# wvu-irl/flope

Hardware: AMD Instinct MI355X
Metric: poses_per_sec (higher is better)
Workload: dtype f16; 1 GPU; PoseResNet (ResNet-18 trunk + fp32 head) forward + special Procrustes + pose assembly, batch 256 x 224x224x3 16-bit NHWC crops resident in HBM per GPU (BASELINE configs[1]); one RCCL all-gather of the poses per run when N>1 (configs[3]); batch_per_gpu=256, global_batch=256, crop=224, parallelism=dp1, weights=synthetic_state_dict(seed 0), eval-mode BN folded

## Files before the change

flope_amd/csrc/conv_s1r.hip:

```cpp
#include "common.h"
#include "plan.h"
#include <type_traits>

namespace {

__device__ __forceinline__ void glds16(const char* gptr, unsigned lds_addr) {
  asm volatile("s_mov_b32 m0, %1\n\ts_nop 0\n\tglobal_load_lds_dwordx4 %0, off" ::"v"(gptr), "s"(lds_addr) : "memory");
}
#define GLDS16(gptr, lptr) glds16((gptr), (unsigned)__builtin_amdgcn_readfirstlane((int)(size_t)(__attribute__((address_space(3))) char*)(lptr)))

template <typename T, bool RES, bool FOLD>
__global__ __launch_bounds__(512, 1) void conv_s1r_kernel(const ConvP p, const u32x4* __restrict__ wpk) {
  static_assert(!(RES && FOLD), "the folded shortcut replaces the residual");
  typedef typename Elem<T>::frag frag;
  constexpr int NPT = 7, WO = 28;
  constexpr int PROW_B = 32 * 64;
  constexpr int IMG_B = 6 * PROW_B;
  constexpr int BUF_B = 4 * IMG_B;
  constexpr int SWAP_OFF = 2 * BUF_B;
  constexpr int NSTEP = 18;
  extern __shared__ __attribute__((aligned(16))) char smem[];

  const int tid = threadIdx.x, lane = tid & 63, wave = tid >> 6, g = lane >> 4, r16 = lane & 15;
  const int cg = wave & 3, kh = wave >> 2;
  const int G = gridDim.x, total = p.B * (p.Ho >> 2), rgs = p.Ho >> 2;

  int dso[4];
  {
    const int px = 16 * (wave & 1) + (lane >> 2);
#pragma unroll
    for (int k = 0; k < 4; ++k) dso[k] = min(px, WO + 1) * 256 + (wave >> 1) * 64 + (((lane & 3) ^ k) << 4);
  }
  const int wrow = p.Wip * 256;
  char* const dbase = smem + (wave >> 1) * IMG_B + (wave & 1) * 1024;
#define S1R_PIECE(src_, buf_, k_) GLDS16((src_) + (k_) * wrow + dso[(k_) & 3], dbase + (buf_) * BUF_B + (k_) * PROW_B)

  const int i8 = r16 < 4 ? r16 : (r16 < 12 ? r16 - 4 : r16 - 8);
  const int rr = i8 >> 1, cc = 2 * (i8 & 1) + ((r16 >= 4 && r16 < 12) ? 1 : 0);
  int rd[3];
#pragma unroll
  for (int dy = 0; dy < 3; ++dy) rd[dy] = kh * 2 * IMG_B + (rr + dy) * PROW_B + cc * 64 + ((g ^ ((rr + dy) & 3)) << 4);
  const int ooff = ((rr * p.Wop + cc) * p.Cout + 32 * cg + 8 * g) * 2;

#ifdef FLOPE_STAG_DBG
  const unsigned long long t_entry_ = __builtin_amdgcn_s_memtime(), rt_entry_ = __builtin_amdgcn_s_memrealtime();
#endif
  int tile = blockIdx.x;
  if (tile >= total) return;
  auto band = [&](int tl) -> const char* {
    tl = min(tl, total - 1);
    const int img = tl / rgs, rg = tl - img * rgs;
    return (const char*)p.in + ((size_t)img * p.Hip + 4 * rg) * p.Wip * 256;
  };
#pragma unroll
  for (int k = 0; k < 6; ++k) S1R_PIECE(band(tile), 0, k);

  const u32x4* const wl = wpk + (size_t)(cg * 2 + kh) * NSTEP * 2 * 64 + lane;
  frag wres[NSTEP][2];
  f32x4 b4[2];
#pragma unroll
  for (int s = 0; s < NSTEP; ++s)
#pragma unroll
    for (int ct = 0; ct < 2; ++ct) wres[s][ct] = __builtin_bit_cast(frag, wl[(s * 2 + ct) * 64]);
#pragma unroll
  for (int ct = 0; ct < 2; ++ct) b4[ct] = *(const f32x4*)(p.bias + 32 * cg + 8 * g + 4 * ct);
  frag wds[2];
  if constexpr (FOLD) {
#pragma unroll
    for (int ct = 0; ct < 2; ++ct) wds[ct] = __builtin_bit_cast(frag, ((const u32x4*)p.ds_w)[((cg * 2 + kh) * 2 + ct) * 64 + lane]);
#pragma unroll
    for (int ct = 0; ct < 2; ++ct) asm volatile("" : "+v"(wds[ct]));
  }
  const int xsoff = FOLD ? ((2 * rr + 1) * p.ds_Wip + 2 * cc + 1) * 128 + kh * 64 + g * 16 : 0;
#pragma unroll
  for (int s = 0; s < NSTEP; ++s)
#pragma unroll
    for (int ct = 0; ct < 2; ++ct) asm volatile("" : "+v"(wres[s][ct]));
#pragma unroll
  for (int ct = 0; ct < 2; ++ct) asm volatile("" : "+v"(b4[ct]));
  asm volatile("s_waitcnt vmcnt(0)" ::: "memory");
  __builtin_amdgcn_s_barrier();

#ifdef FLOPE_STAG_DBG
  const unsigned long long t_loop_ = __builtin_amdgcn_s_memtime();
#endif
  char* const swp = smem + SWAP_OFF + cg * (14 * 1024) + lane * 16;
  const f32x4 zero4 = {0.f, 0.f, 0.f, 0.f};
  int cur = 0;
  const char* nsrc = nullptr;
  const char* xsrc = nullptr;
  size_t opix = 0;

#ifdef FLOPE_STAG_DBG
  unsigned long long stp[12] = {0};
  int st_it = 0;
#define S1R_STAMP(i_) do { if ((p.dbg & 64) && st_it == 1) { __builtin_amdgcn_sched_barrier(0); stp[i_] = __builtin_amdgcn_s_memtime(); __builtin_amdgcn_sched_barrier(0); } } while (0)
#else
#define S1R_STAMP(i_) do {} while (0)
#endif
  auto sub = [&](auto kh_, auto p0_, auto np_) {
    constexpr int KH = decltype(kh_)::value, P0 = decltype(p0_)::value, NP = decltype(np_)::value;
    constexpr bool FIRST = P0 == 0;
    constexpr int NF = KH ? NP - 2 : 2, F0 = KH ? 2 : 0;
    constexpr int NS = NP - NF, S0 = KH ? 0 : 2;
    constexpr int WSLOT = (FIRST ? 0 : 8) + (KH ? (FIRST ? 4 : 2) : 0);
    constexpr int RSLOT = (FIRST ? 0 : 8) + (KH ? 0 : (FIRST ? 4 : 2));
    char* const obase = (char*)p.out + opix;
    const char* const rbase = RES ? (const char*)p.res + opix : nullptr;
    char* const xbuf = smem + cur * BUF_B + P0 * 256;
    const int nbuf = cur ^ 1;
    f32x4 acc[NP][2];
    frag xf[2][NP];
    frag xs[NP];
    S1R_STAMP(FIRST ? 0 : 5);
    auto xaddr = [&](int s) -> const char* {
      const int hc = s / 9, tap = s - 9 * hc, ky = tap / 3, kx = tap - 3 * ky;
      return xbuf + hc * IMG_B + rd[ky] + kx * 64;
    };
#pragma unroll
    for (int pt = 0; pt < NP; ++pt) xf[0][pt] = *(const frag*)(xaddr(0) + pt * 256);
    __builtin_amdgcn_sched_barrier(0);
#pragma unroll
    for (int s = 0; s < NSTEP; ++s) {
#pragma unroll
      for (int pt = 0; pt < NP; ++pt) {
#pragma unroll
        for (int ct = 0; ct < 2; ++ct)
          acc[pt][ct] = Elem<T>::mfma(wres[s][ct], xf[s & 1][pt], s == 0 ? (KH ? zero4 : b4[ct]) : acc[pt][ct]);
        if (s + 1 < NSTEP) xf[(s + 1) & 1][pt] = *(const frag*)(xaddr(s + 1) + pt * 256);
        if (FIRST && s < 3 && pt < 2) S1R_PIECE(nsrc, nbuf, 2 * s + pt);
        if (FOLD && s == 12) xs[pt] = *(const frag*)(xsrc + (P0 + pt) * 1024);
        __builtin_amdgcn_sched_group_barrier(0x008, 2, 0);
        if (s + 1 < NSTEP) __builtin_amdgcn_sched_group_barrier(0x100, 1, 0);
        if ((FIRST && s < 3 && pt < 2) || (FOLD && s == 12)) __builtin_amdgcn_sched_group_barrier(0x020, 1, 0);
      }
    }
    if constexpr (FOLD) {
#pragma unroll
      for (int pt = 0; pt < NP; ++pt)
#pragma unroll
        for (int ct = 0; ct < 2; ++ct) acc[pt][ct] = Elem<T>::mfma(wds[ct], xs[pt], acc[pt][ct]);
    }
    S1R_STAMP(FIRST ? 1 : 6);
#pragma unroll
    for (int i = 0; i < NS; ++i)
#pragma unroll
      for (int ct = 0; ct < 2; ++ct) *(f32x4*)(swp + ((WSLOT + i * 2 + ct) * 64) * 16) = acc[S0 + i][ct];
    u32x4 rq[NF];
    if constexpr (RES) {
#pragma unroll
      for (int i = 0; i < NF; ++i) rq[i] = *(const u32x4*)(rbase + (P0 + F0 + i) * 4 * p.Cout * 2);
    }
    __builtin_amdgcn_sched_barrier(0);
    if constexpr (!FIRST) { if constexpr (RES) asm volatile("s_waitcnt vmcnt(%0)" ::"n"(NF) : "memory"); else asm volatile("s_waitcnt vmcnt(0)" ::: "memory"); }
    asm volatile("s_waitcnt lgkmcnt(0)" ::: "memory");
    __builtin_amdgcn_sched_barrier(0);
    S1R_STAMP(FIRST ? 2 : 7);
#ifdef FLOPE_STAG_DBG
    if ((p.dbg & 64) && st_it == 1 && p.split_ws && lane == 0)
      ((unsigned long long*)p.split_ws)[8192 + (size_t)blockIdx.x * 16 + (FIRST ? 0 : 8) + wave] = __builtin_amdgcn_s_memtime();
#endif
    __builtin_amdgcn_s_barrier();
    __builtin_amdgcn_sched_barrier(0);
    asm volatile("" ::: "memory");
    S1R_STAMP(FIRST ? 3 : 8);
#pragma unroll
    for (int i = 0; i < NF; ++i) {
      u32x4 o;
#pragma unroll
      for (int ct = 0; ct < 2; ++ct) {
        const f32x4 pa = *(const f32x4*)(swp + ((RSLOT + i * 2 + ct) * 64) * 16);
        f32x4 v = KH ? pa + acc[F0 + i][ct] : acc[F0 + i][ct] + pa;
        if constexpr (RES) {
          v[0] += unpack_lo<T>(rq[i][2 * ct]); v[1] += unpack_hi<T>(rq[i][2 * ct]);
          v[2] += unpack_lo<T>(rq[i][2 * ct + 1]); v[3] += unpack_hi<T>(rq[i][2 * ct + 1]);
        }
        o[2 * ct] = pk_out16<T>(pack2<T>(v[0], v[1]), p.relu);
        o[2 * ct + 1] = pk_out16<T>(pack2<T>(v[2], v[3]), p.relu);
      }
      *(u32x4*)(obase + (P0 + F0 + i) * 4 * p.Cout * 2) = o;
    }
    __builtin_amdgcn_sched_barrier(0);
    S1R_STAMP(FIRST ? 4 : 9);
  };
  auto run = [&](auto kh_) {
    for (; tile < total; tile += G) {
      nsrc = band(tile + G);
      const int img = tile / rgs, rg = tile - img * rgs;
      if constexpr (FOLD) xsrc = (const char*)p.ds_in + ((size_t)img * p.ds_Hip + 8 * rg) * p.ds_Wip * 128 + xsoff;
      opix = (((size_t)img * p.Hop + 4 * rg + 1) * p.Wop + 1) * p.Cout * 2 + ooff;
      sub(kh_, std::integral_constant<int, 0>{}, std::integral_constant<int, 4>{});
      sub(kh_, std::integral_constant<int, 4>{}, std::integral_constant<int, 3>{});
#ifdef FLOPE_STAG_DBG
      if ((p.dbg & 64) && st_it == 1 && p.split_ws && tid == 0) {
        unsigned long long* d_ = (unsigned long long*)p.split_ws + (size_t)blockIdx.x * 16;
        for (int i = 0; i < 10; ++i) d_[i] = stp[i];
      }
      ++st_it;
#endif
      cur ^= 1;
    }
  };
  if (kh == 0) run(std::integral_constant<int, 0>{});
  else run(std::integral_constant<int, 1>{});
#ifdef FLOPE_STAG_DBG
  if ((p.dbg & 64) && p.split_ws && tid == 0) {
    unsigned long long* d_ = (unsigned long long*)p.split_ws + (size_t)blockIdx.x * 16;
    d_[10] = t_entry_; d_[11] = t_loop_; d_[12] = __builtin_amdgcn_s_memtime(); d_[13] = rt_entry_; d_[14] = __builtin_amdgcn_s_memrealtime();
  }
#endif
  asm volatile("s_waitcnt vmcnt(0)" ::: "memory");
#undef S1R_PIECE
#undef S1R_STAMP
}

}

extern "C" int flope_conv_s1r_ok(const ConvP* p) { return flope_plan::s1r_ok(flope_plan::dims_of(*p)); }

extern "C" int flope_conv_s1r_lds() { return (int)flope_plan::kS1rLds; }

extern "C" int flope_conv_s1r_init() {
  hipError_t e = hipSuccess;
#define A(T, R, F) if (e == hipSuccess) e = hipFuncSetAttribute((const void*)conv_s1r_kernel<T, R, F>, hipFuncAttributeMaxDynamicSharedMemorySize, flope_conv_s1r_lds());
  A(bf16_t, false, false) A(bf16_t, true, false) A(bf16_t, false, true) A(f16_t, false, false) A(f16_t, true, false) A(f16_t, false, true)
#undef A
  return (int)e;
}

extern "C" int flope_conv_s1r_launch(const ConvP* p, const void* w, int dtype, int grid, void* stream) {
  if (!flope_conv_s1r_ok(p) || !w) return (int)hipErrorInvalidValue;
  const int total = p->B * (p->Ho >> 2);
  if (grid > total) grid = total;
  if (grid < 1) return (int)hipErrorInvalidValue;
  const size_t lds = (size_t)flope_conv_s1r_lds();
  hipStream_t st = (hipStream_t)stream;
#define GO(T) do { if (p->ds_in) hipLaunchKernelGGL((conv_s1r_kernel<T, false, true>), dim3(grid), dim3(512), lds, st, *p, (const u32x4*)w);  \
                   else if (p->res) hipLaunchKernelGGL((conv_s1r_kernel<T, true, false>), dim3(grid), dim3(512), lds, st, *p, (const u32x4*)w);  \
                   else hipLaunchKernelGGL((conv_s1r_kernel<T, false, false>), dim3(grid), dim3(512), lds, st, *p, (const u32x4*)w); } while (0)
  if (dtype == 0) GO(bf16_t); else GO(f16_t);
#undef GO
  return (int)hipGetLastError();
}
```

flope_amd/csrc/engine.hip:

```cpp
#include "../../include/flope_amd.h"
#include "common.h"
#include "host_pack.h"
#include "plan.h"

#include <math.h>
#include <stdio.h>
#include <stdlib.h>
#include <string.h>

#include <map>
#include <string>
#include <vector>

extern "C" int flope_conv_mfma_init();
extern "C" int flope_conv_mfma_launch(const ConvP* p, int dtype, int cfg, int patch, int nbuf, size_t lds, void* stream);
extern "C" int flope_stem_init();
extern "C" int flope_stem_launch(const StemP* p, int dtype, size_t lds, void* stream);
extern "C" int flope_maxpool_launch(const PoolP* p, int dtype, void* stream);
extern "C" int flope_avgpool_launch(const void* in, float* out, int B, int h, int w, int C, int dtype, void* stream);
extern "C" int flope_fc1_launch(const float* feat, const float* W1, const float* W1p, const float* b1, float* hidden, int B, int K, int N, void* stream);
extern "C" int flope_fc2_procrustes_launch(const float* hidden, const float* W2, const float* b2, float* r9, float* R, int B, int K, const float* xyz, int nullify, float* Rt, void* stream);
extern "C" int flope_fc2_procrustes_k4_launch(const float* hidden, const float* W2, const float* b2, float* r9, float* R, int B, int K, const float* xyz, int nullify, float* Rt, void* stream);
extern "C" int flope_prep_input_launch(const void* x, int in_format, int B, int H, int W, void* out, int Hip, int Wip, int dtype, void* stream);
extern "C" int flope_read_stage_launch(const void* in, float* out, int B, int C, int h, int w, int dtype, void* stream);
extern "C" int flope_naive_conv_launch(const NaiveConvP* p, void* stream);
extern "C" int flope_conv_f32m_init();
extern "C" int flope_conv_f32m_launch(const F32mConvP* p, int mp, int stem, int grid, size_t lds, size_t ws_bytes, void* stream);
extern "C" int flope_conv_stag_init();
extern "C" int flope_conv_gstag_init();
extern "C" int flope_conv_w4_init();
extern "C" int flope_conv_r4_init();
extern "C" int flope_conv_r4_launch(const ConvP* p, int dtype, int grid_blocks, void* stream);
extern "C" int flope_conv_s1r_init();
extern "C" int flope_conv_s1r_launch(const ConvP* p, const void* w, int dtype, int grid, void* stream);
extern "C" int flope_conv_s2r_init();
extern "C" int flope_conv_s2r_launch(const ConvP* p, const void* w, int dtype, int grid, void* stream);
extern "C" int flope_conv_w4_launch(const ConvP* p, int dtype, int grid_blocks, int mt, void* stream);
extern "C" int flope_conv_gstag_launch(const ConvP* p, int dtype, void* stream);
extern "C" int flope_conv_stag_launch(const ConvP* p, int dtype, int grid_blocks, size_t lds, void* stream);
extern "C" int flope_conv_split_finalize_launch(const ConvP* p, int dtype, void* stream);
extern "C" int flope_stem_pool_init();
extern "C" int flope_stem_pool_r_blocks_per_cu();
#ifdef FLOPE_STAG_DBG
extern "C" void flope_stem_pool_set_dbg(void* ptr);
#endif
extern "C" int flope_stem_pool_launch(const void* x, int in_format, int B, int H, int W, int Hs, int Ws_, int Hq, int Wq,
                                      const void* w, const void* w2, int* queues, const float* bias, void* out, int dtype, int persist_blocks, void* stream);

using namespace flope_host;
using namespace flope_plan;

namespace {

thread_local std::string g_last_error;

constexpr double kBnEps = 1e-5;
constexpr size_t kDbgRegion = 1 << 20;
constexpr size_t kBufSlack = 1 << 20;

enum Image {
  kWPacked,
  kWStag,
  kWS2r,
  kWS1r,
  kWNaive,
  kWF32m,
  kBias,
  kWDsStag,
  kWDsS1r,
  kBiasFused,
  kImages
};

struct ConvDev {
  int in_buf = -1, out_buf = -1, res_buf = -1;
  int ip_in = -1, ip_out = -1, ip_res = -1;
  void* img[kImages] = {nullptr};
  Launch last;
};

struct Buf { void* ptr = nullptr; size_t bytes = 0; int C = 0, h = 0, w = 0; };

}

struct flope_engine {
  int device = 0, H = 0, W = 0, maxB = 0, dtype = 0, bod = 2048;
  int esz = 2;
  int num_cus = 256;
  PlanOptions opt;
  Plan plan;
  void* stem_in = nullptr; size_t stem_in_bytes = 0;
  int* stem_q = nullptr;
  void* stem_w = nullptr; void* stem_w2 = nullptr; float* stem_w_naive = nullptr; float* stem_w_f32m = nullptr; float* stem_bias = nullptr;
  std::vector<Buf> bufs;
  std::vector<ConvDev> convs;
  int stage_buf[10];
  int mid_buf[8];
  int ds_buf[3] = {-1, -1, -1}, ds_conv[3] = {-1, -1, -1};
  bool last_ds_folded[3] = {false, false, false};
  int final_buf = -1;
  int ip_final = -1;
  int stage_conv[10];
  int mid_conv[8];
  std::vector<int> ip_last_writer;
  bool ip_now = false;
  bool last_inplace = false;
  std::vector<int> last_ip_out, last_ip_writer;
  float *feat = nullptr, *hidden = nullptr, *W1 = nullptr, *W1p = nullptr, *b1 = nullptr, *W2 = nullptr, *b2 = nullptr;
  float* r9_scratch = nullptr;
  bool weights_loaded = false;
  float* split_ws = nullptr; size_t split_ws_bytes = 0;
  hipStream_t side[4] = {nullptr, nullptr, nullptr, nullptr};
  hipEvent_t ev_fork = nullptr, ev_join[4] = {nullptr, nullptr, nullptr, nullptr};
  std::vector<hipEvent_t> ev;
  int ev_n = 0;
  std::vector<int> ev_slice;
  int last_batch = 0;
// ... 434 lines not shown
  const bool fused = o.fuse_stem && dt != FLOPE_DT_F32;
  if (fused) {
    SMARK();
#ifdef FLOPE_STAG_DBG
    flope_stem_pool_set_dbg(((o.dbg & 64) && e->split_ws) ? (void*)(e->split_ws + (size_t)30 * (kDbgRegion / 4)) : nullptr);
#endif
    const bool stem_r = o.stem_r && e->stem_w2 && e->stem_q;
    K_TRY(e, "stem+maxpool", flope_stem_pool_launch(xs, in_format, batch, e->H, e->W, pl.Hs, pl.Ws, pl.Hq, pl.Wq, e->stem_w, stem_r ? e->stem_w2 : nullptr,
                                                   stem_r ? e->stem_q + 1024 * (x.slices > 1 ? x.slice : 0) : nullptr,
                                                   e->stem_bias, pool_out, dt,
                                                   stem_r ? flope_stem_pool_r_blocks_per_cu() * e->num_cus
                                                          : (o.stem_persist == 2 || (o.stem_persist == 1 && pl.Hq * pl.Wq <= 64 * 64)) ? 2 * e->num_cus : 0,
                                                   stream));
  } else {
    SMARK();
    K_TRY(e, "prep_input", flope_prep_input_launch(xs, in_format, batch, e->H, e->W, stem_in, pl.sHip, pl.sWip, dt, stream));
    if (dt == FLOPE_DT_F32 && o.f32mfma) {
      const Launch L = f32m_stem_launch(pl, x);
      F32mConvP p; memset(&p, 0, sizeof(p));
      p.in = (const float*)stem_in; p.out = (float*)stem_out; p.w = e->stem_w_f32m; p.bias = e->stem_bias;
      p.B = batch; p.Hip = pl.sHip; p.Wip = pl.sWip; p.Cin_stored = 4; p.Cin = 3; p.Ho = pl.Hs; p.Wo = pl.Ws;
      p.Hop = pl.Hs + 2; p.Wop = pl.Ws + 2; p.Cout = 64; p.KH = 7; p.KW = 7; p.stride = 2; p.in_off = 0; p.relu = 1;
      p.M = batch * pl.Hs * pl.Ws; p.nsteps = kF32mStemSteps;
      fastdiv_magic((unsigned)(pl.Hs * pl.Ws), &p.mg_hw, &p.sh_hw);
      fastdiv_magic((unsigned)pl.Ws, &p.mg_w, &p.sh_w);
      SMARK();
      K_TRY(e, "stem (fp32 MFMA)", flope_conv_f32m_launch(&p, L.mt, 1, L.grid, L.lds_bytes, 0, stream));
    } else if (dt == FLOPE_DT_F32) {
      NaiveConvP p; memset(&p, 0, sizeof(p));
      p.in = (const float*)stem_in; p.out = (float*)stem_out; p.w = e->stem_w_naive; p.bias = e->stem_bias;
      p.B = batch; p.Hip = pl.sHip; p.Wip = pl.sWip; p.Cin_stored = 4; p.Cin = 3; p.Ho = pl.Hs; p.Wo = pl.Ws;
      p.Hop = pl.Hs + 2; p.Wop = pl.Ws + 2; p.Cout = 64; p.KH = 7; p.KW = 7; p.stride = 2; p.in_off = 0; p.relu = 1;
      SMARK();
      K_TRY(e, "stem (fp32)", flope_naive_conv_launch(&p, stream));
    } else {
      StemP p; memset(&p, 0, sizeof(p));
      p.in = stem_in; p.out = stem_out; p.w = e->stem_w; p.bias = e->stem_bias;
      p.B = batch; p.Hip = pl.sHip; p.Wip = pl.sWip; p.Ho = pl.Hs; p.Wo = pl.Ws;
      p.tiles_per_image = pl.stem_tiles; p.patch_rows_max = pl.stem_rows;
      SMARK();
      K_TRY(e, "stem", flope_stem_launch(&p, dt, pl.stem_lds, stream));
    }
    PoolP pp; pp.in = stem_out; pp.out = pool_out; pp.B = batch; pp.Hip = pl.Hs + 2; pp.Wip = pl.Ws + 2; pp.C = 64; pp.Ho = pl.Hq; pp.Wo = pl.Wq;
    SMARK();
    K_TRY(e, "maxpool", flope_maxpool_launch(&pp, dt, stream));
  }
  for (size_t i = 0; i < e->convs.size(); ++i) {
    ConvDev& c = e->convs[i];
    const ConvShape& s = pl.shape[i];
    const Launch L = decide(o, pl, (int)i, x);
    if (x.slice == x.slices - 1) c.last = L;
    ConvP p, pf;
    if (L.family != kFolded && L.family != kNaive && L.family != kF32m) conv_params(e, (int)i, L, start, batch, &p, &pf);
    if (L.family != kFolded) SMARK();
    switch (L.family) {
      case kFolded: break;
      case kNaive: {
        NaiveConvP q; memset(&q, 0, sizeof(q));
        q.in = (const float*)buf_at(e, in_of(e, c), start); q.out = (float*)buf_at(e, out_of(e, c), start);
        q.res = res_of(e, c) >= 0 ? (const float*)buf_at(e, res_of(e, c), start) : nullptr;
        q.w = (const float*)c.img[kWNaive]; q.bias = (const float*)c.img[kBias];
        q.B = batch; q.Hip = s.hin + 2; q.Wip = s.win + 2; q.Cin_stored = s.cin; q.Cin = s.cin; q.Ho = s.hout; q.Wo = s.wout;
        q.Hop = s.hout + 2; q.Wop = s.wout + 2; q.Cout = s.cout; q.KH = s.k; q.KW = s.k; q.stride = s.stride;
        q.in_off = s.k == 3 ? 0 : 1; q.relu = s.relu;
        K_TRY(e, conv_name(s).c_str(), flope_naive_conv_launch(&q, stream));
        break;
      }
      case kF32m: {
        F32mConvP q; memset(&q, 0, sizeof(q));
        q.in = (const float*)buf_at(e, in_of(e, c), start); q.out = (float*)buf_at(e, out_of(e, c), start);
        q.res = res_of(e, c) >= 0 ? (const float*)buf_at(e, res_of(e, c), start) : nullptr;
        q.w = (const float*)c.img[kWF32m]; q.bias = (const float*)c.img[kBias];
        q.B = batch; q.Hip = s.hin + 2; q.Wip = s.win + 2; q.Cin_stored = s.cin; q.Cin = s.cin; q.Ho = s.hout; q.Wo = s.wout;
        q.Hop = s.hout + 2; q.Wop = s.wout + 2; q.Cout = s.cout; q.KH = s.k; q.KW = s.k; q.stride = s.stride;
        q.in_off = s.k == 3 ? 0 : 1; q.relu = s.relu;
        q.M = batch * s.hout * s.wout; q.csteps = s.cin / 16; q.nsteps = f32m_steps(s.cin, s.k);
        fastdiv_magic((unsigned)(s.hout * s.wout), &q.mg_hw, &q.sh_hw);
        fastdiv_magic((unsigned)s.wout, &q.mg_w, &q.sh_w);
        if (L.ksplit > 1) { q.ksplit = L.ksplit; q.split_ws = e->split_ws; }
        K_TRY(e, conv_name(s).c_str(), flope_conv_f32m_launch(&q, L.mt, 0, L.grid, L.lds_bytes, e->split_ws_bytes, stream));
        break;
      }
      case kGstag: K_TRY(e, conv_name(s).c_str(), flope_conv_gstag_launch(&p, dt, stream)); break;
      case kS1r: K_TRY(e, conv_name(s).c_str(), flope_conv_s1r_launch(&p, c.img[kWS1r], dt, L.grid, stream)); break;
      case kR4: K_TRY(e, conv_name(s).c_str(), flope_conv_r4_launch(&p, dt, L.grid, stream)); break;
      case kW4: K_TRY(e, conv_name(s).c_str(), flope_conv_w4_launch(&p, dt, L.grid, L.mt, stream)); break;
      case kStagFlat: case kStag512x64: case kStagBands:
        K_TRY(e, conv_name(s).c_str(), flope_conv_stag_launch(&p, dt, L.grid, L.lds_bytes, stream));
        if (L.ksplit > 1) K_TRY(e, conv_name(s).c_str(), flope_conv_split_finalize_launch(&pf, dt, stream));
        break;
      case kS2r: K_TRY(e, conv_name(s).c_str(), flope_conv_s2r_launch(&p, c.img[kWS2r], dt, L.grid, stream)); break;
      case kMfma: K_TRY(e, conv_name(s).c_str(), flope_conv_mfma_launch(&p, dt, L.cfg, L.patch, L.nbuf, L.lds_bytes, stream)); break;
    }
  }
  const int final_buf = e->ip_now ? e->ip_final : e->final_buf;
  const Buf& bl = e->bufs[final_buf];
  SMARK();
  K_TRY(e, "avgpool", flope_avgpool_launch(buf_at(e, final_buf, start), feat, batch, bl.h, bl.w, 512, dt, stream));
  SMARK();
  K_TRY(e, "fc1", flope_fc1_launch(feat, e->W1, o.fc1_packed ? e->W1p : nullptr, e->b1, hidden, batch, 512, e->bod, stream));
  if (head) {
    SMARK();
    float* r9 = (r9_dev ? r9_dev : e->r9_scratch) + (size_t)start * 9;
    float* Rp = R_dev ? R_dev + (size_t)start * 9 : nullptr;
    const float* xyzp = po.xyz ? po.xyz + (size_t)start * 3 : nullptr;
    float* Rtp = po.Rt ? po.Rt + (size_t)start * 16 : nullptr;
    int k4 = 0;
    if (o.fc2_k4) {
      k4 = flope_fc2_procrustes_k4_launch(hidden, e->W2, e->b2, r9, Rp, batch, e->bod, xyzp, po.nullify, Rtp, stream);
      if (k4 < 0) return fail(e, FLOPE_EHIP, "fc_rot+procrustes: launch failed");
    }
    if (!k4) K_TRY(e, "fc_rot+procrustes", flope_fc2_procrustes_launch(hidden, e->W2, e->b2, r9, Rp, batch, e->bod, xyzp, po.nullify, Rtp, stream));
  }
  SMARK();
#undef SMARK
  return FLOPE_OK;
}

static int run_trunk(flope_engine* e, const void* x_dev, int in_format, int batch, void* stream, bool head = false,
                     float* r9_dev = nullptr, float* R_dev = nullptr, const PoseOut& po = PoseOut()) {
  if (!e->weights_loaded) return fail(e, FLOPE_ESTATE, "forward before flope_load_weights");
  if (!x_dev) return fail(e, FLOPE_EINVAL, "forward: x_dev is NULL");
  if (batch < 1 || batch > e->maxB) return fail(e, FLOPE_EINVAL, "forward: batch must be within 1..max_batch");
  if (in_format < 0 || in_format > 3) return fail(e, FLOPE_EINVAL, "forward: unknown input format");
  HIP_TRY(e, hipSetDevice(e->device));
  e->ev_n = 0;
  e->last_fused = e->opt.fuse_stem && e->dtype != FLOPE_DT_F32;
  e->last_batch = batch;
  for (int i = 0; i < 3; ++i) e->last_ds_folded[i] = e->ds_conv[i] >= 0 && e->plan.conv[e->ds_conv[i]].folded;
  e->ip_now = e->last_inplace = e->opt.inplace != 0;
  if (e->ip_now) {
    e->last_ip_out.resize(e->convs.size());
    for (size_t i = 0; i < e->convs.size(); ++i) e->last_ip_out[i] = e->convs[i].ip_out;
    e->last_ip_writer = e->ip_last_writer;
  }
  const Slices sl = slices(e->opt, batch, e->opt.profile);
  const int ns = sl.n;
  if (ns == 1) return run_slice(e, x_dev, in_format, 0, slice_ctx(sl, 0, batch, e->num_cus), stream, true, head, r9_dev, R_dev, po);
  hipStream_t user = (hipStream_t)stream;
  if (e->opt.profile == 2) MARK(e, user, 0);
  HIP_TRY(e, hipEventRecord(e->ev_fork, user));
  const int first_side = e->opt.inline0 ? 1 : 0;
  const bool marks = e->opt.profile == 2;
  int rc_all = FLOPE_OK, forked = first_side;
  for (int s = first_side; s < ns && rc_all == FLOPE_OK; ++s) {
    if (hipStreamWaitEvent(e->side[s], e->ev_fork, 0) != hipSuccess) { rc_all = fail(e, FLOPE_EHIP, "hipStreamWaitEvent(fork) failed"); break; }

    forked = s + 1;
    if (e->opt.lag && !e->opt.inline0 && s == ns - 1 && batch >= 192) {
      hipLaunchKernelGGL(lag_kernel, dim3(1), dim3(64), 0, e->side[s], e->opt.lag);
      if (hipGetLastError() != hipSuccess) { rc_all = fail(e, FLOPE_EHIP, "lag kernel launch failed"); break; }
    }
    rc_all = run_slice(e, x_dev, in_format, sl.start[s], slice_ctx(sl, s, batch, e->num_cus), e->side[s], marks, head, r9_dev, R_dev, po);
  }
  if (e->opt.inline0 && rc_all == FLOPE_OK)
    rc_all = run_slice(e, x_dev, in_format, sl.start[0], slice_ctx(sl, 0, batch, e->num_cus), user, marks, head, r9_dev, R_dev, po);
  const std::string first_err = rc_all != FLOPE_OK ? e->err : std::string();
  for (int s = first_side; s < forked; ++s) {
    if (hipEventRecord(e->ev_join[s], e->side[s]) != hipSuccess || hipStreamWaitEvent(user, e->ev_join[s], 0) != hipSuccess) {
      hipStreamSynchronize(e->side[s]);
      if (rc_all == FLOPE_OK) rc_all = fail(e, FLOPE_EHIP, "joining the batch-slice streams failed");
    }
  }
  if (rc_all != FLOPE_OK) {
    if (!first_err.empty()) { e->err = first_err; g_last_error = first_err; }
    e->last_batch = 0;
  }
// ... 120 lines not shown
```

flope_amd/csrc/plan.h:

```cpp
#pragma once

#include "../../include/flope_amd.h"
#include "w4_sched.h"

#include <limits.h>
#include <stdio.h>
#include <string.h>

#include <algorithm>
#include <string>
#include <vector>

namespace flope_plan {

constexpr size_t kLdsTwoBlocks = 80 * 1024;
constexpr size_t kLdsMax = 160 * 1024;
constexpr size_t kGstagLds = 3 * 32768 + 3 * 16384;
constexpr size_t kR4Lds = (size_t)2 * 5 * 8192 + 18 * 4096 + 4 * 2048;
constexpr size_t kS1rLds = 2 * 4 * 6 * 32 * 64 + 4 * 14 * 1024;
constexpr size_t kS2rLds = 2 * 18 * 32 * 128;
constexpr size_t kF32mLds = kLdsTwoBlocks + 4096;

struct PlanOptions {
  int patch = 1;
  int bm256 = 1;
  int persist = 0;
  int rows_grid = 0;
  int split = 0;
  int fc1_packed = 1;
  int w4mtlo = 0;
  int lag = 20;
  int w4mt = 0;
  int fc2_k4 = 1;
  int ksplit = 1;
  int stem_r = 1;
  int stem_persist = 1;
  int rowseg = 1;
  int skew = 1;
  int r4 = 1;
  int s1r = 1;
  int s2r_grid = 0;
  int s2r = 1;
  int w4 = 1;
  int w4cw = 4;
  int w4cwf = 0;
  int prio = 0;
  int reslds = 1;
  int gstag = 1;
  int dsfuse = 1;
  int stag = 3;
  int streams = 2;
  int fuse_stem = 1;
  int ldspad = 0;
  int dbg = 0;
  int nbuf = 2;
  int f32mfma = 0;
  int f32m_ksplit = 0;
  int inline0 = 1;
  int inplace = 0;
  int profile = 0;
};

enum OptionKind { kBool, kClamp, kMask, kInOrZero, kZeroOrClamp, kNbuf };
struct OptionDef { const char* name; int PlanOptions::*member; OptionKind kind; int lo, hi; bool replans; };

inline const std::vector<OptionDef>& option_table() {
  typedef PlanOptions O;
  static const std::vector<OptionDef> t = {
      {"patch", &O::patch, kBool, 0, 1, true},
      {"bm256", &O::bm256, kBool, 0, 1, true},
      {"persist", &O::persist, kBool, 0, 1, false},
      {"rows_grid", &O::rows_grid, kClamp, -1, INT_MAX, false},
      {"split", &O::split, kClamp, 0, INT_MAX, false},
      {"fc1_packed", &O::fc1_packed, kBool, 0, 1, false},
      {"w4mtlo", &O::w4mtlo, kZeroOrClamp, 5, 8, false},
      {"lag", &O::lag, kClamp, 0, 500, false},
      {"w4mt", &O::w4mt, kInOrZero, 5, 8, false},
      {"fc2_k4", &O::fc2_k4, kBool, 0, 1, false},
      {"ksplit", &O::ksplit, kClamp, 0, 2, false},
      {"stem_r", &O::stem_r, kBool, 0, 1, false},
      {"stem_persist", &O::stem_persist, kClamp, 0, 2, false},
      {"rowseg", &O::rowseg, kBool, 0, 1, true},
      {"skew", &O::skew, kBool, 0, 1, true},
      {"r4", &O::r4, kBool, 0, 1, false},
      {"s1r", &O::s1r, kBool, 0, 1, false},
      {"s2r_grid", &O::s2r_grid, kClamp, INT_MIN, INT_MAX, false},
      {"s2r", &O::s2r, kBool, 0, 1, false},
      {"w4", &O::w4, kBool, 0, 1, false},
      {"w4cw", &O::w4cw, kClamp, 0, 64, false},
      {"w4cwf", &O::w4cwf, kMask, 0, 3, false},
      {"prio", &O::prio, kClamp, 0, 2, false},
      {"reslds", &O::reslds, kBool, 0, 1, false},
      {"gstag", &O::gstag, kClamp, 0, 2, true},
      {"dsfuse", &O::dsfuse, kBool, 0, 1, true},
      {"stag", &O::stag, kClamp, 0, 3, true},
      {"streams", &O::streams, kClamp, 1, 4, false},
      {"fuse_stem", &O::fuse_stem, kBool, 0, 1, false},
      {"ldspad", &O::ldspad, kClamp, INT_MIN, INT_MAX, false},
      {"dbg", &O::dbg, kClamp, INT_MIN, INT_MAX, false},
      {"nbuf", &O::nbuf, kNbuf, 2, 3, true},
      {"profile", &O::profile, kClamp, 0, 2, false},
      {"f32mfma", &O::f32mfma, kBool, 0, 1, false},
      {"f32m_ksplit", &O::f32m_ksplit, kClamp, 0, 32, false},
      {"inline0", &O::inline0, kBool, 0, 1, false},
      {"inplace", &O::inplace, kBool, 0, 1, false},
  };
  return t;
}

inline const OptionDef* find_option(const char* name) {
  for (const OptionDef& d : option_table())
    if (std::string(d.name) == name) return &d;
  return nullptr;
}

inline int set_option(PlanOptions& o, const char* name, int value, bool* replan) {
  const OptionDef* d = find_option(name);
  if (replan) *replan = d && d->replans;
  if (!d) return FLOPE_EINVAL;
  const int prev = o.*(d->member);
  const int clamped = value < d->lo ? d->lo : (value > d->hi ? d->hi : value);
  int v = clamped;
  switch (d->kind) {
    case kBool: v = value != 0; break;
    case kClamp: break;
    case kMask: v = value & d->hi; break;
    case kInOrZero: v = clamped == value ? value : 0; break;
    case kZeroOrClamp: v = value <= 0 ? 0 : clamped; break;
    case kNbuf: v = value == 2 ? 2 : 3; break;
  }
  o.*(d->member) = v;
  return prev;
}

enum ConvRole { kConv1, kShortcut, kConv2 };
struct ConvShape {
  int li = 0, bi = 0, role = kConv1;
  int cin = 0, cout = 0, k = 0, stride = 1;
  int hin = 0, win = 0, hout = 0, wout = 0;
  int res = 0;
  int relu = 0;
};

inline std::string conv_name(const ConvShape& s, bool bn = false) {
  const std::string p = "base.layer" + std::to_string(s.li) + "." + std::to_string(s.bi);
  if (s.role == kShortcut) return p + (bn ? ".downsample.1" : ".downsample.0");
  return p + (bn ? ".bn" : ".conv") + (s.role == kConv1 ? "1" : "2");
}

inline bool has_stag_image(const ConvShape& s) { return s.k == 3 && s.cin % 64 == 0; }
inline bool has_s1r_image(const ConvShape& s) { return s.k == 3 && s.stride == 1 && s.cin == 128 && s.cout == 128; }
inline bool has_s2r_image(const ConvShape& s) { return s.k == 3 && s.stride == 2 && s.cin == 64 && s.cout == 128; }
inline bool has_ds_s1r_image(const ConvShape& s) { return s.k == 1 && s.stride == 2 && s.cin == 64 && s.cout == 128; }
inline bool has_ds_stag_image(const ConvShape& s) { return s.k == 1 && s.cout >= 128 && s.cin % 64 == 0; }

inline int out_dim(int n, int k, int s, int p) { return (n + 2 * p - k) / s + 1; }

struct ConvDims {
  int stride, ntaps, Cin, Cout, Ho, Wo, Hip, Wip, ksplit;
  bool res, ds, ds_w;
  int ds_Cin, ds_Hip, ds_Wip;
};
template <typename P>
inline ConvDims dims_of(const P& p) {
  return {p.stride, p.ntaps, p.Cin, p.Cout, p.Ho, p.Wo, p.Hip, p.Wip, p.ksplit, p.res != nullptr, p.ds_in != nullptr, p.ds_w != nullptr,
          p.ds_Cin, p.ds_Hip, p.ds_Wip};
}
inline bool r4_ok(const ConvDims& p) {
  return p.stride == 1 && p.ntaps == 9 && p.Cin == 64 && p.Cout == 64 && p.Wo == 56 && p.Ho % 8 == 0 &&
         10 * (p.Wip + 2) * 4 <= 5 * 512 && p.ksplit <= 1 && !p.ds;
}
inline bool s1r_ok(const ConvDims& p) {
  if (p.ds && !(p.ds_Cin == 64 && p.ds_Hip == 2 * p.Ho + 2 && p.ds_Wip == 2 * p.Wo + 2 && p.ds_w && !p.res)) return false;
  return p.stride == 1 && p.ntaps == 9 && p.Cin == 128 && p.Cout == 128 && p.Wo == 28 && (p.Ho & 3) == 0 &&
         p.ksplit <= 1 && p.Wip == p.Wo + 2 && p.Hip == p.Ho + 2;
}
inline bool s2r_ok(const ConvDims& p) {
  return p.stride == 2 && p.ntaps == 9 && p.Cin == 64 && p.Cout == 128 && p.Wo == 28 && (p.Ho & 3) == 0 && !p.res && !p.ds &&
         p.ksplit <= 1 && p.Wip == 2 * p.Wo + 2 && p.Hip == 2 * p.Ho + 2;
}
inline size_t w4_lds(int pt, int mt, int dsf, int pers) {
  if (pt < 4 || pt > 6 || mt < 5 || mt > 8 || (mt < 7 && pt != 4) || (pers && (mt != 7 || pt > 5))) return 0;
  return w4_lds_bytes(pt, dsf && pers);
}

struct ConvPlan {
  int cfg = 0, patch = 0, nbuf = 2, per_image = 0, tiles_per_image = 0, ntiles = 0, rows_max = 0;
  size_t lds = 0;
// ... 482 lines not shown
```

Measured before the change: 275,900 poses/s.

## Peel first tile in s1r conv to stream weights and move prefetch to kh=1 waves

Adds a YW template mode to the stride-1 resident conv kernel and makes mode 2 the default. In that mode the first tile is peeled so only the first few weight steps are loaded before the loop, and the rest (plus the fused downsample weights) stream in during the first tile's MFMA steps. This is meant to hide the cold-start weight-load latency. The next band's prefetch is also moved out of the interleaved MFMA loop into one 12-piece burst issued by the kh=1 waves, which drops the vmcnt wait for kh=0 waves. The cost is more template variants, a more complex schedule, and possible register-pressure or ordering hazards in the peeled path.

After: 278,900 poses/s (median of 6 runs). 1.01x the previous value.

```diff
diff --git a/flope_amd/csrc/conv_s1r.hip b/flope_amd/csrc/conv_s1r.hip
--- a/flope_amd/csrc/conv_s1r.hip
+++ b/flope_amd/csrc/conv_s1r.hip
@@ -9,7 +9,7 @@
 }
 #define GLDS16(gptr, lptr) glds16((gptr), (unsigned)__builtin_amdgcn_readfirstlane((int)(size_t)(__attribute__((address_space(3))) char*)(lptr)))
 
-template <typename T, bool RES, bool FOLD>
+template <typename T, bool RES, bool FOLD, int YW>
 __global__ __launch_bounds__(512, 1) void conv_s1r_kernel(const ConvP p, const u32x4* __restrict__ wpk) {
   static_assert(!(RES && FOLD), "the folded shortcut replaces the residual");
   typedef typename Elem<T>::frag frag;
@@ -19,6 +19,8 @@
   constexpr int BUF_B = 4 * IMG_B;
   constexpr int SWAP_OFF = 2 * BUF_B;
   constexpr int NSTEP = 18;
+  constexpr bool PEEL = YW == 2;
+  constexpr int WD = 4;
   extern __shared__ __attribute__((aligned(16))) char smem[];
 
   const int tid = threadIdx.x, lane = tid & 63, wave = tid >> 6, g = lane >> 4, r16 = lane & 15;
@@ -34,6 +36,10 @@
   const int wrow = p.Wip * 256;
   char* const dbase = smem + (wave >> 1) * IMG_B + (wave & 1) * 1024;
 #define S1R_PIECE(src_, buf_, k_) GLDS16((src_) + (k_) * wrow + dso[(k_) & 3], dbase + (buf_) * BUF_B + (k_) * PROW_B)
+  const int ypx0 = (lane >> 2) * 256 + (wave & 3) * 64, ypx1 = min(16 + (lane >> 2), WO + 1) * 256 + (wave & 3) * 64, ysl = (lane & 3) << 4;
+  char* const ybase = smem + (wave & 3) * IMG_B;
+#define S1R_YPIECE(src_, buf_, q_) GLDS16((src_) + ((q_) >> 1) * wrow + (((q_) & 1) ? ypx1 : ypx0) + (ysl ^ ((((q_) >> 1) & 3) << 4)), \
+                                          ybase + (buf_) * BUF_B + ((q_) >> 1) * PROW_B + ((q_) & 1) * 1024)
 
   const int i8 = r16 < 4 ? r16 : (r16 < 12 ? r16 - 4 : r16 - 8);
   const int rr = i8 >> 1, cc = 2 * (i8 & 1) + ((r16 >= 4 && r16 < 12) ? 1 : 0);
@@ -54,31 +60,46 @@
   };
 #pragma unroll
   for (int k = 0; k < 6; ++k) S1R_PIECE(band(tile), 0, k);
+  if constexpr (PEEL) asm volatile("s_waitcnt vmcnt(0)" ::: "memory");
 
   const u32x4* const wl = wpk + (size_t)(cg * 2 + kh) * NSTEP * 2 * 64 + lane;
   frag wres[NSTEP][2];
   f32x4 b4[2];
-#pragma unroll
-  for (int s = 0; s < NSTEP; ++s)
+  if constexpr (PEEL) {
+#pragma unroll
+    for (int ct = 0; ct < 2; ++ct) b4[ct] = *(const f32x4*)(p.bias + 32 * cg + 8 * g + 4 * ct);
+  }
+#pragma unroll
+  for (int s = 0; s < (PEEL ? WD : NSTEP); ++s)
 #pragma unroll
     for (int ct = 0; ct < 2; ++ct) wres[s][ct] = __builtin_bit_cast(frag, wl[(s * 2 + ct) * 64]);
-#pragma unroll
-  for (int ct = 0; ct < 2; ++ct) b4[ct] = *(const f32x4*)(p.bias + 32 * cg + 8 * g + 4 * ct);
+  if constexpr (!PEEL) {
+#pragma unroll
+    for (int ct = 0; ct < 2; ++ct) b4[ct] = *(const f32x4*)(p.bias + 32 * cg + 8 * g + 4 * ct);
+  }
   frag wds[2];
-  if constexpr (FOLD) {
-#pragma unroll
-    for (int ct = 0; ct < 2; ++ct) wds[ct] = __builtin_bit_cast(frag, ((const u32x4*)p.ds_w)[((cg * 2 + kh) * 2 + ct) * 64 + lane]);
+  const u32x4* const wdl = FOLD ? (const u32x4*)p.ds_w + (size_t)(cg * 2 + kh) * 2 * 64 + lane : nullptr;
+  if constexpr (FOLD && !PEEL) {
+#pragma unroll
+    for (int ct = 0; ct < 2; ++ct) wds[ct] = __builtin_bit_cast(frag, wdl[ct * 64]);
 #pragma unroll
     for (int ct = 0; ct < 2; ++ct) asm volatile("" : "+v"(wds[ct]));
   }
   const int xsoff = FOLD ? ((2 * rr + 1) * p.ds_Wip + 2 * cc + 1) * 128 + kh * 64 + g * 16 : 0;
-#pragma unroll
-  for (int s = 0; s < NSTEP; ++s)
-#pragma unroll
-    for (int ct = 0; ct < 2; ++ct) asm volatile("" : "+v"(wres[s][ct]));
-#pragma unroll
-  for (int ct = 0; ct < 2; ++ct) asm volatile("" : "+v"(b4[ct]));
-  asm volatile("s_waitcnt vmcnt(0)" ::: "memory");
+  auto settle = [&]() {
+    if constexpr (FOLD && PEEL) {
+#pragma unroll
+      for (int ct = 0; ct < 2; ++ct) asm volatile("" : "+v"(wds[ct]));
+    }
+#pragma unroll
+    for (int s = 0; s < NSTEP; ++s)
+#pragma unroll
+      for (int ct = 0; ct < 2; ++ct) asm volatile("" : "+v"(wres[s][ct]));
+#pragma unroll
+    for (int ct = 0; ct < 2; ++ct) asm volatile("" : "+v"(b4[ct]));
+  };
+  if constexpr (!PEEL) { settle(); asm volatile("s_waitcnt vmcnt(0)" ::: "memory"); }
+  __builtin_amdgcn_sched_barrier(0);
   __builtin_amdgcn_s_barrier();
 
 #ifdef FLOPE_STAG_DBG
@@ -98,9 +119,11 @@
 #else
 #define S1R_STAMP(i_) do {} while (0)
 #endif
-  auto sub = [&](auto kh_, auto p0_, auto np_) {
+  auto sub = [&](auto kh_, auto p0_, auto np_, auto peeled_) {
     constexpr int KH = decltype(kh_)::value, P0 = decltype(p0_)::value, NP = decltype(np_)::value;
     constexpr bool FIRST = P0 == 0;
+    constexpr bool YHEAD = decltype(peeled_)::value ? !FIRST : FIRST;
+    constexpr bool WLOAD = decltype(peeled_)::value && FIRST;
     constexpr int NF = KH ? NP - 2 : 2, F0 = KH ? 2 : 0;
     constexpr int NS = NP - NF, S0 = KH ? 0 : 2;
     constexpr int WSLOT = (FIRST ? 0 : 8) + (KH ? (FIRST ? 4 : 2) : 0);
@@ -119,6 +142,10 @@
     };
 #pragma unroll
     for (int pt = 0; pt < NP; ++pt) xf[0][pt] = *(const frag*)(xaddr(0) + pt * 256);
+    if constexpr (YW >= 1 && KH == 1 && YHEAD) {
+#pragma unroll
+      for (int q = 0; q < 12; ++q) S1R_YPIECE(nsrc, nbuf, q);
+    }
     __builtin_amdgcn_sched_barrier(0);
 #pragma unroll
     for (int s = 0; s < NSTEP; ++s) {
@@ -128,11 +155,14 @@
         for (int ct = 0; ct < 2; ++ct)
           acc[pt][ct] = Elem<T>::mfma(wres[s][ct], xf[s & 1][pt], s == 0 ? (KH ? zero4 : b4[ct]) : acc[pt][ct]);
         if (s + 1 < NSTEP) xf[(s + 1) & 1][pt] = *(const frag*)(xaddr(s + 1) + pt * 256);
-        if (FIRST && s < 3 && pt < 2) S1R_PIECE(nsrc, nbuf, 2 * s + pt);
+        if (YW == 0 && FIRST && s < 3 && pt < 2) S1R_PIECE(nsrc, nbuf, 2 * s + pt);
         if (FOLD && s == 12) xs[pt] = *(const frag*)(xsrc + (P0 + pt) * 1024);
+        if (WLOAD && s + WD < NSTEP && pt < 2) wres[s + WD][pt] = __builtin_bit_cast(frag, wl[((s + WD) * 2 + pt) * 64]);
+        if (WLOAD && FOLD && s + WD == NSTEP && pt < 2) wds[pt] = __builtin_bit_cast(frag, wdl[pt * 64]);
         __builtin_amdgcn_sched_group_barrier(0x008, 2, 0);
         if (s + 1 < NSTEP) __builtin_amdgcn_sched_group_barrier(0x100, 1, 0);
-        if ((FIRST && s < 3 && pt < 2) || (FOLD && s == 12)) __builtin_amdgcn_sched_group_barrier(0x020, 1, 0);
+        if ((YW == 0 && FIRST && s < 3 && pt < 2) || (FOLD && s == 12)) __builtin_amdgcn_sched_group_barrier(0x020, 1, 0);
+        if (WLOAD && pt < 2 && (s + WD < NSTEP || (FOLD && s + WD == NSTEP))) __builtin_amdgcn_sched_group_barrier(0x020, 1, 0);
       }
     }
     if constexpr (FOLD) {
@@ -152,7 +182,7 @@
       for (int i = 0; i < NF; ++i) rq[i] = *(const u32x4*)(rbase + (P0 + F0 + i) * 4 * p.Cout * 2);
     }
     __builtin_amdgcn_sched_barrier(0);
-    if constexpr (!FIRST) { if constexpr (RES) asm volatile("s_waitcnt vmcnt(%0)" ::"n"(NF) : "memory"); else asm volatile("s_waitcnt vmcnt(0)" ::: "memory"); }
+    if constexpr (!FIRST && (YW == 0 || KH == 1)) { if constexpr (RES) asm volatile("s_waitcnt vmcnt(%0)" ::"n"(NF) : "memory"); else asm volatile("s_waitcnt vmcnt(0)" ::: "memory"); }
     asm volatile("s_waitcnt lgkmcnt(0)" ::: "memory");
     __builtin_amdgcn_sched_barrier(0);
     S1R_STAMP(FIRST ? 2 : 7);
@@ -183,17 +213,17 @@
     __builtin_amdgcn_sched_barrier(0);
     S1R_STAMP(FIRST ? 4 : 9);
   };
-  auto run = [&](auto kh_) {
-    for (; tile < total; tile += G) {
+  auto one = [&](auto kh_, auto peeled_) {
+    {
       nsrc = band(tile + G);
       const int img = tile / rgs, rg = tile - img * rgs;
       if constexpr (FOLD) xsrc = (const char*)p.ds_in + ((size_t)img * p.ds_Hip + 8 * rg) * p.ds_Wip * 128 + xsoff;
       opix = (((size_t)img * p.Hop + 4 * rg + 1) * p.Wop + 1) * p.Cout * 2 + ooff;
-      sub(kh_, std::integral_constant<int, 0>{}, std::integral_constant<int, 4>{});
-      sub(kh_, std::integral_constant<int, 4>{}, std::integral_constant<int, 3>{});
-#ifdef FLOPE_STAG_DBG
-      if ((p.dbg & 64) && st_it == 1 && p.split_ws && tid == 0) {
-        unsigned long long* d_ = (unsigned long long*)p.split_ws + (size_t)blockIdx.x * 16;
+      sub(kh_, std::integral_constant<int, 0>{}, std::integral_constant<int, 4>{}, peeled_);
+      sub(kh_, std::integral_constant<int, 4>{}, std::integral_constant<int, 3>{}, peeled_);
+#ifdef FLOPE_STAG_DBG
+      if ((p.dbg & 64) && st_it == 1 && p.split_ws && (tid == 0 || tid == 256)) {
+        unsigned long long* d_ = (unsigned long long*)p.split_ws + (tid ? 16384 : 0) + (size_t)blockIdx.x * 16;
         for (int i = 0; i < 10; ++i) d_[i] = stp[i];
       }
       ++st_it;
@@ -201,6 +231,15 @@
       cur ^= 1;
     }
   };
+  auto run = [&](auto kh_) {
+    if constexpr (PEEL) {
+      one(kh_, std::true_type{});
+      tile += G;
+      __builtin_amdgcn_sched_barrier(0);
+      settle();
+    }
+    for (; tile < total; tile += G) one(kh_, std::false_type{});
+  };
   if (kh == 0) run(std::integral_constant<int, 0>{});
   else run(std::integral_constant<int, 1>{});
 #ifdef FLOPE_STAG_DBG
@@ -211,6 +250,7 @@
 #endif
   asm volatile("s_waitcnt vmcnt(0)" ::: "memory");
 #undef S1R_PIECE
+#undef S1R_YPIECE
 #undef S1R_STAMP
 }
 
@@ -222,23 +262,27 @@
 
 extern "C" int flope_conv_s1r_init() {
   hipError_t e = hipSuccess;
-#define A(T, R, F) if (e == hipSuccess) e = hipFuncSetAttribute((const void*)conv_s1r_kernel<T, R, F>, hipFuncAttributeMaxDynamicSharedMemorySize, flope_conv_s1r_lds());
+#define A1(T, R, F, Y) if (e == hipSuccess) e = hipFuncSetAttribute((const void*)conv_s1r_kernel<T, R, F, Y>, hipFuncAttributeMaxDynamicSharedMemorySize, flope_conv_s1r_lds());
+#define A(T, R, F) A1(T, R, F, 0) A1(T, R, F, 1) A1(T, R, F, 2)
   A(bf16_t, false, false) A(bf16_t, true, false) A(bf16_t, false, true) A(f16_t, false, false) A(f16_t, true, false) A(f16_t, false, true)
 #undef A
+#undef A1
   return (int)e;
 }
 
-extern "C" int flope_conv_s1r_launch(const ConvP* p, const void* w, int dtype, int grid, void* stream) {
+extern "C" int flope_conv_s1r_launch(const ConvP* p, const void* w, int dtype, int grid, int yw, void* stream) {
   if (!flope_conv_s1r_ok(p) || !w) return (int)hipErrorInvalidValue;
   const int total = p->B * (p->Ho >> 2);
   if (grid > total) grid = total;
   if (grid < 1) return (int)hipErrorInvalidValue;
   const size_t lds = (size_t)flope_conv_s1r_lds();
   hipStream_t st = (hipStream_t)stream;
-#define GO(T) do { if (p->ds_in) hipLaunchKernelGGL((conv_s1r_kernel<T, false, true>), dim3(grid), dim3(512), lds, st, *p, (const u32x4*)w);  \
-                   else if (p->res) hipLaunchKernelGGL((conv_s1r_kernel<T, true, false>), dim3(grid), dim3(512), lds, st, *p, (const u32x4*)w);  \
-                   else hipLaunchKernelGGL((conv_s1r_kernel<T, false, false>), dim3(grid), dim3(512), lds, st, *p, (const u32x4*)w); } while (0)
-  if (dtype == 0) GO(bf16_t); else GO(f16_t);
+#define GO(T, Y) do { if (p->ds_in) hipLaunchKernelGGL((conv_s1r_kernel<T, false, true, Y>), dim3(grid), dim3(512), lds, st, *p, (const u32x4*)w);  \
+                      else if (p->res) hipLaunchKernelGGL((conv_s1r_kernel<T, true, false, Y>), dim3(grid), dim3(512), lds, st, *p, (const u32x4*)w);  \
+                      else hipLaunchKernelGGL((conv_s1r_kernel<T, false, false, Y>), dim3(grid), dim3(512), lds, st, *p, (const u32x4*)w); } while (0)
+#define GOY(T) do { if (yw == 1) GO(T, 1); else if (yw == 2) GO(T, 2); else GO(T, 0); } while (0)
+  if (dtype == 0) GOY(bf16_t); else GOY(f16_t);
+#undef GOY
 #undef GO
   return (int)hipGetLastError();
 }
diff --git a/flope_amd/csrc/engine.hip b/flope_amd/csrc/engine.hip
--- a/flope_amd/csrc/engine.hip
+++ b/flope_amd/csrc/engine.hip
@@ -32,7 +32,7 @@
 extern "C" int flope_conv_r4_init();
 extern "C" int flope_conv_r4_launch(const ConvP* p, int dtype, int grid_blocks, void* stream);
 extern "C" int flope_conv_s1r_init();
-extern "C" int flope_conv_s1r_launch(const ConvP* p, const void* w, int dtype, int grid, void* stream);
+extern "C" int flope_conv_s1r_launch(const ConvP* p, const void* w, int dtype, int grid, int yw, void* stream);
 extern "C" int flope_conv_s2r_init();
 extern "C" int flope_conv_s2r_launch(const ConvP* p, const void* w, int dtype, int grid, void* stream);
 extern "C" int flope_conv_w4_launch(const ConvP* p, int dtype, int grid_blocks, int mt, void* stream);
@@ -633,7 +633,7 @@
         break;
       }
       case kGstag: K_TRY(e, conv_name(s).c_str(), flope_conv_gstag_launch(&p, dt, stream)); break;
-      case kS1r: K_TRY(e, conv_name(s).c_str(), flope_conv_s1r_launch(&p, c.img[kWS1r], dt, L.grid, stream)); break;
+      case kS1r: K_TRY(e, conv_name(s).c_str(), flope_conv_s1r_launch(&p, c.img[kWS1r], dt, L.grid, o.coldyw, stream)); break;
       case kR4: K_TRY(e, conv_name(s).c_str(), flope_conv_r4_launch(&p, dt, L.grid, stream)); break;
       case kW4: K_TRY(e, conv_name(s).c_str(), flope_conv_w4_launch(&p, dt, L.grid, L.mt, stream)); break;
       case kStagFlat: case kStag512x64: case kStagBands:
diff --git a/flope_amd/csrc/plan.h b/flope_amd/csrc/plan.h
--- a/flope_amd/csrc/plan.h
+++ b/flope_amd/csrc/plan.h
@@ -58,6 +58,7 @@
   int f32m_ksplit = 0;
   int inline0 = 1;
   int inplace = 0;
+  int coldyw = 2;
   int profile = 0;
 };
 
@@ -104,6 +105,7 @@
       {"f32m_ksplit", &O::f32m_ksplit, kClamp, 0, 32, false},
       {"inline0", &O::inline0, kBool, 0, 1, false},
       {"inplace", &O::inplace, kBool, 0, 1, false},
+      {"coldyw", &O::coldyw, kClamp, 0, 2, false},
   };
   return t;
 }
```
